# IGNF/MAESTRO

Hardware: AMD Instinct MI355X
Metric: MAE-pretrain tiles/sec (higher is better)
Workload: dtype bf16

## Files before the change

### maestro_amd/csrc/gemm.hip

```cpp
#include "gemm_reg.hpp"

namespace {

template <bool A_KMAJOR, bool B_KMAJOR, int MT = 4>
__global__ __launch_bounds__(NT, MT == 2 ? 3 : 2) void gemm_kernel(GemmParams p) {
    static_assert(!A_KMAJOR || MT == 4, "the K-major A image is 128 columns wide");
    constexpr int TBM = 32 * MT, NA = MT;
    constexpr int A_BYTES = TBM * 128, B_BYTES = TILE_BYTES;
    __shared__ __attribute__((aligned(16))) unsigned char smem[2 * A_BYTES + 2 * B_BYTES];
    unsigned char* const sb = smem + 2 * A_BYTES;
    const int nwg = p.tiles_m * p.tiles_n;
    const int id = xcd_remap(blockIdx.x, nwg);
    constexpr int GROUP_M = MT == 2 ? 16 : 8;
    int tile_m, tile_n;
    raster_tile<GROUP_M>(p, id, tile_m, tile_n);
    const int m0 = tile_m * TBM, n0 = tile_n * BN;
    const int kbeg = blockIdx.y * p.k_per_split;
    const int kend = min(p.K, kbeg + p.k_per_split);
    const int nk = (kend - kbeg + BK - 1) / BK;

    const int w = threadIdx.x >> 6, l = threadIdx.x & 63;
    const int wm = (w >> 1) * (16 * MT), wn = (w & 1) * 64;

    f32x4 acc[4][MT];
#pragma unroll
    for (int j = 0; j < 4; ++j)
#pragma unroll
        for (int i = 0; i < MT; ++i) acc[j][i] = (f32x4){0.f, 0.f, 0.f, 0.f};

    u32x4 ra[NA], rb[4];
    auto mfma_block = [&](const bf16x8 (&fa)[MT], const bf16x8 (&fb)[4]) {
#pragma unroll
        for (int j = 0; j < 4; ++j)
#pragma unroll
            for (int i = 0; i < MT; ++i)
                acc[j][i] = __builtin_amdgcn_mfma_f32_16x16x32_bf16(fb[j], fa[i], acc[j][i], 0, 0, 0);
    };
    auto compute = [&](const unsigned char* ta, const unsigned char* tb) {
#pragma unroll
        for (int s = 0; s < 2; ++s) {
            bf16x8 fa[MT], fb[4];
#pragma unroll
            for (int i = 0; i < MT; ++i) fa[i] = read_frag<A_KMAJOR>(ta, wm + 16 * i, s);
#pragma unroll
            for (int j = 0; j < 4; ++j) fb[j] = read_frag<B_KMAJOR>(tb, wn + 16 * j, s);
            mfma_block(fa, fb);
        }
    };
    auto compute_half = [&](const unsigned char* ta, const unsigned char* tb, int s) {
        bf16x8 fa[MT], fb[4];
#pragma unroll
        for (int i = 0; i < MT; ++i) fa[i] = read_frag<A_KMAJOR>(ta, wm + 16 * i, s);
#pragma unroll
        for (int j = 0; j < 4; ++j) fb[j] = read_frag<B_KMAJOR>(tb, wn + 16 * j, s);
        __builtin_amdgcn_s_setprio(1);
        mfma_block(fa, fb);
        __builtin_amdgcn_s_setprio(0);
    };
    if (p.fast) {
        const __amdgpu_buffer_rsrc_t ra_src = buffer_rsrc(p.A, (int)p.a_bytes);
        const __amdgpu_buffer_rsrc_t rb_src = buffer_rsrc(p.B, (int)p.b_bytes);
        int va[NA], vb[4];
        tile_offsets<A_KMAJOR, NA>(p.lda, m0, va);
        tile_offsets<B_KMAJOR>(p.ldb, n0, vb);
        const int a_step = A_KMAJOR ? BK * p.lda * 2 : BK * 2;
        const int b_step = B_KMAJOR ? BK * p.ldb * 2 : BK * 2;
        int a_off = A_KMAJOR ? kbeg * p.lda * 2 : kbeg * 2;
        int b_off = B_KMAJOR ? kbeg * p.ldb * 2 : kbeg * 2;
        load_tile_fast(ra_src, va, a_off, ra);
        load_tile_fast(rb_src, vb, b_off, rb);
        store_tile<A_KMAJOR, NA>(smem, ra);
        store_tile<B_KMAJOR>(sb, rb);
        if (nk > 1) {
            a_off += a_step; b_off += b_step;
            load_tile_fast(ra_src, va, a_off, ra);
            load_tile_fast(rb_src, vb, b_off, rb);
        }
        __syncthreads();
        constexpr int NM = 4 * MT, NS = NA + 4;
        constexpr int NR = (A_KMAJOR ? 8 : MT) + (B_KMAJOR ? 8 : 4);
        int kt0 = 0;
        for (; kt0 + 2 < nk; ++kt0) {
            const int cur = kt0 & 1;
            const unsigned char* ta = smem + cur * A_BYTES;
            const unsigned char* tb = sb + cur * B_BYTES;
            bf16x8 fa[MT], fb[4];
#pragma unroll
            for (int i = 0; i < MT; ++i) fa[i] = read_frag<A_KMAJOR>(ta, wm + 16 * i, 0);
#pragma unroll
            for (int j = 0; j < 4; ++j) fb[j] = read_frag<B_KMAJOR>(tb, wn + 16 * j, 0);
            mfma_block(fa, fb);
            store_tile<A_KMAJOR, NA>(smem + (cur ^ 1) * A_BYTES, ra);
            store_tile<B_KMAJOR>(sb + (cur ^ 1) * B_BYTES, rb);
            a_off += a_step; b_off += b_step;
            load_tile_fast(ra_src, va, a_off, ra);
            load_tile_fast(rb_src, vb, b_off, rb);
#pragma unroll
            for (int i = 0; i < MT; ++i) fa[i] = read_frag<A_KMAJOR>(ta, wm + 16 * i, 1);
#pragma unroll
            for (int j = 0; j < 4; ++j) fb[j] = read_frag<B_KMAJOR>(tb, wn + 16 * j, 1);
            mfma_block(fa, fb);
            __builtin_amdgcn_sched_group_barrier(0x100, NR, 0);
#pragma unroll
            for (int r = 0; r < NS; ++r) {
                __builtin_amdgcn_sched_group_barrier(0x008, NM / NS, 0);
                __builtin_amdgcn_sched_group_barrier(0x200, 1, 0);
                __builtin_amdgcn_sched_group_barrier(0x020, 1, 0);
            }
            if constexpr (NM % NS != 0) __builtin_amdgcn_sched_group_barrier(0x008, NM - (NM / NS) * NS, 0);
            __builtin_amdgcn_sched_group_barrier(0x100, NR, 0);
            __builtin_amdgcn_sched_group_barrier(0x008, NM, 0);
            __syncthreads();
        }
        for (int kt = kt0; kt < nk; ++kt) {
            const int cur = kt & 1;
            const unsigned char* ta = smem + cur * A_BYTES;
            const unsigned char* tb = sb + cur * B_BYTES;
            compute_half(ta, tb, 0);
            if (kt + 1 < nk) {
                store_tile<A_KMAJOR, NA>(smem + (cur ^ 1) * A_BYTES, ra);
                store_tile<B_KMAJOR>(sb + (cur ^ 1) * B_BYTES, rb);
                if (kt + 2 < nk) {
                    a_off += a_step; b_off += b_step;
                    load_tile_fast(ra_src, va, a_off, ra);
                    load_tile_fast(rb_src, vb, b_off, rb);
                }
            }
            compute_half(ta, tb, 1);
            __syncthreads();
        }
    } else {
        unsigned char* ta = smem;
        unsigned char* tb = sb;
        load_tile<A_KMAJOR, NA>(p.A, p.lda, m0, p.M, kbeg, kend, ra);
        load_tile<B_KMAJOR>(p.B, p.ldb, n0, p.N, kbeg, kend, rb);
        store_tile<A_KMAJOR, NA>(ta, ra);
        store_tile<B_KMAJOR>(tb, rb);
        __syncthreads();
        for (int kt = 0; kt < nk; ++kt) {
            const bool more = kt + 1 < nk;
            if (more) {
                load_tile<A_KMAJOR, NA>(p.A, p.lda, m0, p.M, kbeg + (kt + 1) * BK, kend, ra);
                load_tile<B_KMAJOR>(p.B, p.ldb, n0, p.N, kbeg + (kt + 1) * BK, kend, rb);
            }
            compute(ta, tb);
            __syncthreads();
            if (more) {
                store_tile<A_KMAJOR, NA>(ta, ra);
                store_tile<B_KMAJOR>(tb, rb);
            }
            __syncthreads();
        }
    }

    float* st = reinterpret_cast<float*>(smem) + w * (32 * 68);
    if (p.flags & MH_GEMM_ATOMIC) gemm_epilogue_atomic<MT>(p, acc, st, m0 + wm, n0 + wn);
    else gemm_epilogue_store<MT>(p, acc, st, m0 + wm, n0 + wn);
}

}

static int gemm_reg_launch(int tile, int layout, GemmParams& p, hipStream_t s) {
    const int K = p.K;
    const int mt = tile == MH_TILE_REG_64 ? 2 : tile == MH_TILE_REG_192 ? 6 : 4;
    const int tbm = 32 * mt;
    p.tiles_m = ceil_div(p.M, tbm); p.tiles_n = ceil_div(p.N, BN);
    const int ksteps = ceil_div(K, BK);
    const SplitK sk = (p.flags & MH_GEMM_ATOMIC) ? split_k(p.tiles_m * p.tiles_n, ksteps, 512, 4) : SplitK{ksteps, 1};
    p.k_per_split = sk.ksteps_per * BK;
    const bool a_kmajor = layout == 2, b_kmajor = layout != 0;
    const long k_rows = (long)ksteps * BK;
    const bool tail_ok = (a_kmajor && b_kmajor) || K % BK == 0;
    p.fast = tail_ok && gemm_in_reach((a_kmajor ? k_rows : (long)p.tiles_m * tbm) * p.lda * 2, 4096) &&
             gemm_in_reach((b_kmajor ? k_rows : (long)p.tiles_n * BN) * p.ldb * 2, 4096);
    gemm_set_extents(p, layout);
    dim3 grid(p.tiles_m * p.tiles_n, sk.splits), block(NT);
    for_layout(layout, [&](auto a_kmajor_c, auto b_kmajor_c) {
        constexpr bool AK = decltype(a_kmajor_c)::value, BKM = decltype(b_kmajor_c)::value;
        if (AK || mt == 4) hipLaunchKernelGGL((gemm_kernel<AK, BKM, 4>), grid, block, 0, s, p);
        else if (mt == 2) hipLaunchKernelGGL((gemm_kernel<false, BKM, 2>), grid, block, 0, s, p);
        else hipLaunchKernelGGL((gemm_kernel<false, BKM, 6>), grid, block, 0, s, p);
    });
    MH_LAUNCH_CHECK();
    return 0;
}

static int gemm_check_args(bool buffers, int tile, int layout, const GemmParams& p) {
    const int M = p.M, N = p.N, K = p.K, lda = p.lda, ldb = p.ldb, ldc = p.ldc, ldr = p.ldr, ldaux = p.ldaux, flags = p.flags;
    auto given = [&](const void* q) { return !buffers || q; };
    MH_CHECK_ARG(tile >= MH_TILE_AUTO && tile <= MH_TILE_REG_192, "mh_gemm_bf16: tile %d", tile);
    MH_CHECK_ARG(layout >= 0 && layout <= 2, "mh_gemm_bf16: layout %d", layout);
    MH_CHECK_ARG(!(flags & ~0x7ff), "mh_gemm_bf16: unknown flag bits 0x%x", flags & ~0x7ff);
    MH_CHECK_ARG(M > 0 && N > 0 && K > 0, "mh_gemm_bf16: empty problem %d %d %d", M, N, K);
    MH_CHECK_ARG(given(p.A) && given(p.B) && given(p.C), "mh_gemm_bf16: null operand");
    MH_CHECK_ARG(lda % 8 == 0 && ldb % 8 == 0, "mh_gemm_bf16: lda/ldb must be multiples of 8 (%d, %d)", lda, ldb);
    MH_CHECK_ARG(N % 4 == 0 && ldc % 4 == 0, "mh_gemm_bf16: N and ldc must be multiples of 4 (%d, %d)", N, ldc);
    MH_CHECK_ARG((flags & MH_GEMM_OUT_F32) || (N % 8 == 0 && ldc % 8 == 0), "mh_gemm_bf16: bf16 output needs N, ldc %% 8 == 0");
    MH_CHECK_ARG((flags & MH_GEMM_OUT_F32) || !(flags & MH_GEMM_RESIDUAL), "mh_gemm_bf16: residual epilogue needs f32 output");
    MH_CHECK_ARG(!(flags & MH_GEMM_OUT_F32) || !(flags & (MH_GEMM_GELU | MH_GEMM_DGELU | MH_GEMM_MULAUX)), "mh_gemm_bf16: GELU / aux epilogues need bf16 output");
    MH_CHECK_ARG(((uintptr_t)p.A | (uintptr_t)p.B | (uintptr_t)p.C) % 16 == 0, "mh_gemm_bf16: bases must be 16-B aligned");
    if (layout == 2) {
        MH_CHECK_ARG(M % 8 == 0 && N % 8 == 0, "mh_gemm_bf16: TN needs M, N multiples of 8 (%d, %d)", M, N);
    } else {
        MH_CHECK_ARG(K % 8 == 0, "mh_gemm_bf16: K must be a multiple of 8 (%d)", K);
        if (layout == 1) MH_CHECK_ARG(N % 8 == 0, "mh_gemm_bf16: NN needs N multiple of 8 (%d)", N);
    }
    MH_CHECK_ARG(!(flags & MH_GEMM_BIAS) || given(p.bias), "mh_gemm_bf16: bias flag without pointer");
    MH_CHECK_ARG(!(flags & MH_GEMM_RESIDUAL) || (given(p.res) && ldr % 4 == 0), "mh_gemm_bf16: residual needs pointer, ldr%%4==0");
    MH_CHECK_ARG(!(flags & (MH_GEMM_DGELU | MH_GEMM_MULAUX)) || (given(p.aux_in) && ldaux % 8 == 0), "mh_gemm_bf16: dgelu / mulaux need aux_in, ldaux %% 8 == 0");
    MH_CHECK_ARG(!(flags & MH_GEMM_AUX_DGELU) || ((flags & MH_GEMM_GELU) && given(p.aux_out)), "mh_gemm_bf16: aux_dgelu needs the GELU epilogue and aux_out");
    MH_CHECK_ARG(!((flags & MH_GEMM_DGELU) && (flags & MH_GEMM_MULAUX)), "mh_gemm_bf16: dgelu and mulaux exclude each other");
    MH_CHECK_ARG(!(flags & MH_GEMM_AUX_U8) || ((flags & (MH_GEMM_AUX_DGELU | MH_GEMM_MULAUX)) && !(flags & MH_GEMM_DGELU)),
                 "mh_gemm_bf16: MH_GEMM_AUX_U8 applies to the saved GELU derivative only (AUX_DGELU / MULAUX)");
    MH_CHECK_ARG(!(flags & MH_GEMM_GELU) || !p.aux_out || ldaux % 8 == 0, "mh_gemm_bf16: ldaux %% 8");
    MH_CHECK_ARG(!(flags & MH_GEMM_ATOMIC) || (flags & MH_GEMM_OUT_F32), "mh_gemm_bf16: atomic needs f32 output");
    MH_CHECK_ARG(!(flags & MH_GEMM_COLSUM) || (given(p.colsum) && !(flags & MH_GEMM_OUT_F32)), "mh_gemm_bf16: colsum needs a pointer and bf16 output");
    MH_CHECK_ARG(!(flags & MH_GEMM_ATOMIC) || !(flags & ~(MH_GEMM_ATOMIC | MH_GEMM_OUT_F32)),
                 "mh_gemm_bf16: atomic accumulate excludes other epilogues");
    return 0;
}

static bool prefer_dma(int layout, int M, int N, int K, int flags) {
    if (layout == 2 || (flags & MH_GEMM_ATOMIC) || K % 32 != 0 || K < 256) return false;
    const long tiles = (long)ceil_div(M, 256) * ceil_div(N, 256);
    if (tiles < 256) return false;
    const long waves = (tiles + 255) / 256;
    return 10 * tiles >= 9 * 256 * waves;
}

static int gemm_resolve(int tile, int families, int layout, const GemmParams& p) {
    const int M = p.M, N = p.N, K = p.K, flags = p.flags;
    if (tile >= MH_TILE_PP_128 && tile <= MH_TILE_PP_128_DIAG5) return gemm_pp_serves(tile, layout, p) ? tile : -2;
    if (tile > MH_TILE_REG_128 && tile < MH_TILE_PP_128) return gemm_dma_serves(tile, layout, p) ? tile : -2;
    if (tile != MH_TILE_AUTO)
        return layout != 2 && !(flags & MH_GEMM_COLSUM) ? tile : MH_TILE_REG_128;
    const bool dma = (families & MH_GEMM_FAMILY_DMA) && prefer_dma(layout, M, N, K, flags);
    const long t128 = (long)ceil_div(M, 128) * ceil_div(N, 128);
    if ((families & MH_GEMM_FAMILY_192) && !dma && layout != 2 && !(flags & (MH_GEMM_COLSUM | MH_GEMM_ATOMIC)) && K >= 1536 &&
        K % BK == 0 && t128 > 512 && t128 <= 576 && (long)ceil_div(M, 192) * ceil_div(N, 128) <= 512)
        return MH_TILE_REG_192;
    if ((families & MH_GEMM_FAMILY_PP) && !(flags & MH_GEMM_MULAUX) && layout == 0 && t128 >= 256 &&
        ((flags & MH_GEMM_GELU) ? t128 <= 2304 : (!dma || (K < 1024 && t128 <= 8192))) && gemm_pp_serves(MH_TILE_PP_128, layout, p))
        return MH_TILE_PP_128;
    if (dma && gemm_dma_serves(MH_TILE_DMA_256, layout, p)) return MH_TILE_DMA_256;
    return MH_TILE_REG_128;
}

extern "C" int mh_gemm_bf16_resolve_tile(int tile, int families, int layout, int M, int N, int K, int lda, int ldb, int ldc,
                                         int ldr, int ldaux, int flags) {
    GemmParams p;
    gemm_fill(p, M, N, K, nullptr, lda, nullptr, ldb, nullptr, ldc, flags, nullptr, nullptr, ldr, nullptr, nullptr, ldaux, nullptr);
    MH_CHECK_ARG(!(families & ~MH_GEMM_FAMILY_ALL), "mh_gemm_bf16_resolve_tile: unknown family bits 0x%x", families & ~MH_GEMM_FAMILY_ALL);
    if (const int rc = gemm_check_args(false, tile, layout, p)) return rc;
    return gemm_resolve(tile, families, layout, p);
}

extern "C" int mh_gemm_bf16_tile(int tile, int layout, int M, int N, int K, const void* A, int lda, const void* B, int ldb,
                                 void* C, int ldc, int flags, const float* bias, const float* res, int ldr,
                                 const void* aux_in, void* aux_out, int ldaux, float* colsum, void* stream) {
    GemmParams p;
    gemm_fill(p, M, N, K, A, lda, B, ldb, C, ldc, flags, bias, res, ldr, aux_in, aux_out, ldaux, colsum);
    if (const int rc = gemm_check_args(true, tile, layout, p)) return rc;
    const int run = gemm_resolve(tile, MH_GEMM_FAMILY_ALL, layout, p);
    if (run == -2) return -2;
    if (run >= MH_TILE_PP_128 && run <= MH_TILE_PP_128_DIAG5) return gemm_pp_launch(run, layout, p, (hipStream_t)stream);
    if (run > MH_TILE_REG_128 && run < MH_TILE_PP_128) return gemm_dma_launch(run, layout, p, (hipStream_t)stream);
    return gemm_reg_launch(run, layout, p, (hipStream_t)stream);
}

extern "C" int mh_gemm_bf16(int layout, int M, int N, int K, const void* A, int lda, const void* B, int ldb, void* C,
                            int ldc, int flags, const float* bias, const float* res, int ldr, const void* aux_in,
                            void* aux_out, int ldaux, float* colsum, void* stream) {
    return mh_gemm_bf16_tile(MH_TILE_AUTO, layout, M, N, K, A, lda, B, ldb, C, ldc, flags, bias, res, ldr, aux_in, aux_out,
                             ldaux, colsum, stream);
}
```

### maestro_amd/csrc/gemm_common.hpp

```cpp
#pragma once
#include "common.hpp"
#include "../../include/maestro_hip.h"

struct GemmParams {
    const bf16_t* A; const bf16_t* B; void* C;
    const float* bias; const float* res; const bf16_t* aux_in; bf16_t* aux_out; float* colsum;
    int M, N, K, lda, ldb, ldc, ldr, ldaux, flags;
    int tiles_m, tiles_n, k_per_split;
    int fast;
    unsigned a_bytes, b_bytes;
    const float* descale_a = nullptr; const float* descale_b = nullptr;
    uint8_t* c8 = nullptr; const float* c8_scale = nullptr; float* c8_amax = nullptr; int ldc8 = 0;
    const uint8_t* sa = nullptr; const uint8_t* sb = nullptr; int ldsa = 0, ldsb = 0; unsigned sa_bytes = 0, sb_bytes = 0;
    uint8_t* c8_scales = nullptr; int ldc8s = 0;
};

__device__ __forceinline__ __amdgpu_buffer_rsrc_t buffer_rsrc(const void* ptr, int bytes) {
    return __builtin_amdgcn_make_buffer_rsrc((void*)ptr, (short)0, bytes, 0x00020000);
}
__host__ __device__ __forceinline__ long matrix_bytes(int rows, int cols, int ld, int esize) { return ((long)(rows - 1) * ld + cols) * esize; }
__device__ __forceinline__ void swap16(uint32_t& a, uint32_t& b) {
    const u32x2 r = __builtin_amdgcn_permlane16_swap(a, b, false, false);
    a = r[0]; b = r[1];
}
template <int N>
__device__ __forceinline__ void wait_vmcnt() { asm volatile("s_waitcnt vmcnt(%0)" ::"n"(N) : "memory"); }
__device__ __forceinline__ int lane_id() { return __builtin_amdgcn_mbcnt_hi(~0u, __builtin_amdgcn_mbcnt_lo(~0u, 0u)); }
__device__ __forceinline__ int lane_id_opaque() {
    int lane = lane_id();
    asm volatile("" : "+v"(lane));
    return lane;
}
__device__ __forceinline__ int kmajor_sw(int k) { return (k & 3) | (((k >> 3) & 1) << 2); }

template <int GROUP_M>
__device__ __forceinline__ void raster_tile(const GemmParams& p, int id, int& tile_m, int& tile_n) {
    const int per_group = GROUP_M * p.tiles_n;
    const int group = id / per_group, in_group = id - group * per_group;
    const int first_m = group * GROUP_M;
    const int gsz = min(p.tiles_m - first_m, GROUP_M);
    tile_m = first_m + in_group % gsz;
    int n = in_group / gsz;
    const int groups = (p.tiles_m + GROUP_M - 1) / GROUP_M;
    n += ((group * 8) / groups) * p.tiles_n / 8;
    tile_n = n >= p.tiles_n ? n - p.tiles_n : n;
}

__device__ __forceinline__ u32x2 pack_fp8x8(f32x4 lo, f32x4 hi, float s, bool e5m2 = false) {
    const float lim = e5m2 ? 57344.f : 448.f;
#pragma unroll
    for (int e = 0; e < 4; ++e) {
        lo[e] = fminf(fmaxf(lo[e] * s, -lim), lim);
        hi[e] = fminf(fmaxf(hi[e] * s, -lim), lim);
    }
    int a, b;
    if (e5m2) {
        a = __builtin_amdgcn_cvt_pk_bf8_f32(lo[0], lo[1], 0, false);
        a = __builtin_amdgcn_cvt_pk_bf8_f32(lo[2], lo[3], a, true);
        b = __builtin_amdgcn_cvt_pk_bf8_f32(hi[0], hi[1], 0, false);
        b = __builtin_amdgcn_cvt_pk_bf8_f32(hi[2], hi[3], b, true);
    } else {
        a = __builtin_amdgcn_cvt_pk_fp8_f32(lo[0], lo[1], 0, false);
        a = __builtin_amdgcn_cvt_pk_fp8_f32(lo[2], lo[3], a, true);
        b = __builtin_amdgcn_cvt_pk_fp8_f32(hi[0], hi[1], 0, false);
        b = __builtin_amdgcn_cvt_pk_fp8_f32(hi[2], hi[3], b, true);
    }
    return (u32x2){(uint32_t)a, (uint32_t)b};
}
__device__ __forceinline__ uint32_t pack_e4m3x4(f32x4 v, float s) {
#pragma unroll
    for (int e = 0; e < 4; ++e) v[e] = fminf(fmaxf(v[e] * s, -448.f), 448.f);
    int a = __builtin_amdgcn_cvt_pk_fp8_f32(v[0], v[1], 0, false);
    a = __builtin_amdgcn_cvt_pk_fp8_f32(v[2], v[3], a, true);
    return (uint32_t)a;
}
__device__ __forceinline__ uint32_t mx_scale_byte(float a) {
    const uint32_t u = __float_as_uint(a);
    if (u >= 0x7f800000u) return 0xffu;
    if (u == 0u) return 127u;
    const int eb = (int)(u >> 23);
    const int b = eb - 8 + ((u & 0x7fffffu) > 0x600000u ? 1 : 0);
    return eb == 0 ? 0u : (uint32_t)max(b, 0);
}
__device__ __forceinline__ float mx_inv_scale(uint32_t byte) { return byte == 0xffu ? 1.f : __uint_as_float((254u - byte) << 23); }
template <int LANES>
__device__ __forceinline__ float group_amax(float v) {
    uint32_t u = __float_as_uint(v);
#pragma unroll
    for (int o = 1; o < LANES; o <<= 1) u = max(u, (uint32_t)__shfl_xor((int)u, o, 64));
    return __uint_as_float(u);
}

__device__ __forceinline__ void atomic_max_pos(float* row, float v) {
    const unsigned k = ((blockIdx.x + blockIdx.y * gridDim.x) * (blockDim.x >> 6) + (threadIdx.x >> 6)) & (MH_FP8_AMAX_SUBSLOTS - 1);
    __hip_atomic_fetch_max(reinterpret_cast<int*>(row) + k * MH_FP8_AMAX_STRIDE, __float_as_int(v), __ATOMIC_RELAXED,
                           __HIP_MEMORY_SCOPE_AGENT);
}

__host__ __device__ static inline void gemm_fill(GemmParams& p, int M, int N, int K, const void* A, int lda, const void* B, int ldb, void* C, int ldc,
                             int flags, const float* bias, const float* res, int ldr, const void* aux_in, void* aux_out, int ldaux,
                             float* colsum) {
    p.A = (const bf16_t*)A; p.B = (const bf16_t*)B; p.C = C;
    p.bias = bias; p.res = res; p.aux_in = (const bf16_t*)aux_in; p.aux_out = (bf16_t*)aux_out; p.colsum = colsum;
    p.M = M; p.N = N; p.K = K; p.lda = lda; p.ldb = ldb; p.ldc = ldc; p.ldr = ldr; p.ldaux = ldaux; p.flags = flags;
}
__host__ __device__ static inline long gemm_extent(bool kmajor, int rows, int K, int ld, int esize = 2) {
    return kmajor ? matrix_bytes(K, rows, ld, esize) : matrix_bytes(rows, K, ld, esize);
}
static inline void gemm_set_extents(GemmParams& p, int layout) {
    p.a_bytes = (unsigned)gemm_extent(layout == 2, p.M, p.K, p.lda);
    p.b_bytes = (unsigned)gemm_extent(layout != 0, p.N, p.K, p.ldb);
}
static inline bool gemm_in_reach(long bytes, long margin = 65536) { return bytes < (1L << 31) - margin; }
struct SplitK { int ksteps_per, splits; };
static inline SplitK split_k(int tiles, int ksteps, int slots, int min_ksteps) {
    const int want = max(1, min(min(slots / max(tiles, 1), ksteps / min_ksteps), 32));
    const int ksteps_per = ceil_div(ksteps, want);
    return {ksteps_per, ceil_div(ksteps, ksteps_per)};
}
template <class F>
static void for_layout(int layout, F&& fn) {
    using std::false_type; using std::true_type;
    switch (layout) {
        case 0: fn(false_type{}, false_type{}); break;
        case 1: fn(false_type{}, true_type{}); break;
        default: fn(true_type{}, true_type{}); break;
    }
}

bool gemm_dma_serves(int tile, int layout, const GemmParams& p);
int gemm_dma_launch(int tile, int layout, GemmParams& p, hipStream_t stream);
bool gemm_pp_serves(int tile, int layout, const GemmParams& p);
int gemm_pp_launch(int tile, int layout, GemmParams& p, hipStream_t stream);

__device__ __forceinline__ u32x2 pack_dgelu_u8x8(f32x4 lo, f32x4 hi) {
    unsigned a = 0, b = 0;
#pragma unroll
    for (int e = 0; e < 4; ++e) {
        a = __builtin_amdgcn_cvt_pk_u8_f32(__builtin_fmaf(lo[e], 200.f, 26.f), e, a);
        b = __builtin_amdgcn_cvt_pk_u8_f32(__builtin_fmaf(hi[e], 200.f, 26.f), e, b);
    }
    return (u32x2){a, b};
}
__device__ __forceinline__ f32x4 unpack_dgelu_u8x4(unsigned w) {
    return (f32x4){__builtin_fmaf((float)(w & 0xffu), 0.005f, -0.13f), __builtin_fmaf((float)((w >> 8) & 0xffu), 0.005f, -0.13f),
                   __builtin_fmaf((float)((w >> 16) & 0xffu), 0.005f, -0.13f), __builtin_fmaf((float)(w >> 24), 0.005f, -0.13f)};
}

template <int MT, int RP = 32, bool MX = false>
__device__ __forceinline__ void gemm_epilogue_store(const GemmParams& p, const f32x4 (&acc)[4][MT], float* st, int m_base,
                                                    int n_base) {
    constexpr int TPP = RP / 16, NPASS = MT / TPP, SUB = RP / 8;
    static_assert((RP == 16 || RP == 32) && MT % TPP == 0, "staging pass geometry");
    const int l = threadIdx.x & 63, g = l >> 4, lm = l & 15;
    const bool out_f32 = p.flags & MH_GEMM_OUT_F32;
    const float alpha = p.descale_a ? *p.descale_a * *p.descale_b : 1.f;
    if (out_f32) {
        f32x4 bias4[4];
#pragma unroll
        for (int j = 0; j < 4; ++j) {
            const int n = n_base + 16 * j + 4 * g;
            bias4[j] = (f32x4){0, 0, 0, 0};
            if ((p.flags & MH_GEMM_BIAS) && n < p.N) bias4[j] = *reinterpret_cast<const f32x4*>(p.bias + n);
        }
        constexpr int IB = MT % 4 == 0 ? 4 : MT % 3 == 0 ? 3 : MT;
        static_assert(MT % IB == 0, "row blocks per wave");
#pragma unroll
        for (int i0 = 0; i0 < MT; i0 += IB) {
            f32x4 add[IB][4];
#pragma unroll
            for (int ii = 0; ii < IB; ++ii) {
                const int m = m_base + 16 * (i0 + ii) + lm;
#pragma unroll
                for (int j = 0; j < 4; ++j) {
                    const int n = n_base + 16 * j + 4 * g;
                    add[ii][j] = bias4[j];
                    if ((p.flags & MH_GEMM_RESIDUAL) && m < p.M && n < p.N)
                        add[ii][j] += *reinterpret_cast<const f32x4*>(p.res + (size_t)m * p.ldr + n);
                }
            }
#pragma unroll
            for (int ii = 0; ii < IB; ++ii) {
                const int m = m_base + 16 * (i0 + ii) + lm;
#pragma unroll
                for (int j = 0; j < 4; ++j) {
                    const int n = n_base + 16 * j + 4 * g;
                    if (m < p.M && n < p.N)
                        *reinterpret_cast<f32x4*>(reinterpret_cast<float*>(p.C) + (size_t)m * p.ldc + n) = acc[j][i0 + ii] * alpha + add[ii][j];
                }
            }
        }
        return;
    }
    f32x4 cs_lo = {0, 0, 0, 0}, cs_hi = {0, 0, 0, 0};
    float s8 = 0.f;
    if constexpr (!MX) s8 = p.c8 ? *p.c8_scale : 0.f;
    float amax8 = 0.f;
    u32x4 aux_all[NPASS][SUB];
    {
        const int n = n_base + (l & 7) * 8;
        if (p.flags & (MH_GEMM_DGELU | MH_GEMM_MULAUX)) {
#pragma unroll
            for (int pass_m = 0; pass_m < NPASS; ++pass_m)
#pragma unroll
                for (int pass = 0; pass < SUB; ++pass) {
                    const int m = m_base + RP * pass_m + pass * 8 + (l >> 3);
                    aux_all[pass_m][pass] = (u32x4){0, 0, 0, 0};
                    if (m < p.M && n < p.N) {
                        if (p.flags & MH_GEMM_AUX_U8) {
                            const u32x2 b8 = *reinterpret_cast<const u32x2*>(reinterpret_cast<const uint8_t*>(p.aux_in) + (size_t)m * p.ldaux + n);
                            aux_all[pass_m][pass] = (u32x4){b8[0], b8[1], 0, 0};
                        } else {
                            aux_all[pass_m][pass] = *reinterpret_cast<const u32x4*>(p.aux_in + (size_t)m * p.ldaux + n);
                        }
                    }
                }
        }
    }
#pragma unroll
    for (int pass_m = 0; pass_m < NPASS; ++pass_m) {
#pragma unroll
        for (int i = TPP * pass_m; i < TPP * pass_m + TPP; ++i)
#pragma unroll
            for (int j = 0; j < 4; ++j)
                *reinterpret_cast<f32x4*>(st + (16 * (i - TPP * pass_m) + lm) * 68 + 16 * j + 4 * g) = acc[j][i];
        {
            const int c = (l & 7) * 8, n = n_base + c;
            f32x4 b_lo = {0, 0, 0, 0}, b_hi = {0, 0, 0, 0};
            if ((p.flags & MH_GEMM_BIAS) && n < p.N) {
                b_lo = *reinterpret_cast<const f32x4*>(p.bias + n);
                b_hi = *reinterpret_cast<const f32x4*>(p.bias + n + 4);
            }
            const u32x4 (&aux_pre)[SUB] = aux_all[pass_m];
#pragma unroll
            for (int pass = 0; pass < SUB; ++pass) {
                const int r = pass * 8 + (l >> 3), m = m_base + RP * pass_m + r;
                f32x4 lo = *reinterpret_cast<const f32x4*>(st + r * 68 + c);
                f32x4 hi = *reinterpret_cast<const f32x4*>(st + r * 68 + c + 4);
                if (m < p.M && n < p.N) {
                    if (p.descale_a) { lo = lo * alpha + b_lo; hi = hi * alpha + b_hi; }
                    else { lo += b_lo; hi += b_hi; }
                    if (p.flags & MH_GEMM_GELU) {
                        f32x4 c_lo, d_lo, c_hi, d_hi;
                        gelu_cdf_pdf4(lo, c_lo, d_lo);
                        gelu_cdf_pdf4(hi, c_hi, d_hi);
                        if (p.aux_out) {
                            f32x4 a_lo = lo, a_hi = hi;
                            if (p.flags & MH_GEMM_AUX_DGELU) { a_lo = lo * d_lo + c_lo; a_hi = hi * d_hi + c_hi; }
                            if (p.flags & MH_GEMM_AUX_U8) {
                                *reinterpret_cast<u32x2*>(reinterpret_cast<uint8_t*>(p.aux_out) + (size_t)m * p.ldaux + n) =
                                    pack_dgelu_u8x8(a_lo, a_hi);
                            } else {
                                u32x4 pk = {pack_bf2(a_lo[0], a_lo[1]), pack_bf2(a_lo[2], a_lo[3]), pack_bf2(a_hi[0], a_hi[1]),
                                            pack_bf2(a_hi[2], a_hi[3])};
                                *reinterpret_cast<u32x4*>(p.aux_out + (size_t)m * p.ldaux + n) = pk;
                            }
                        }
                        lo *= c_lo; hi *= c_hi;
                    }
                    if (p.flags & MH_GEMM_MULAUX) {
                        const u32x4 pk = aux_pre[pass];
                        if (p.flags & MH_GEMM_AUX_U8) {
                            lo *= unpack_dgelu_u8x4(pk[0]);
                            hi *= unpack_dgelu_u8x4(pk[1]);
                        } else {
                            lo *= bf2x2_to_f32x4(pk[0], pk[1]);
                            hi *= bf2x2_to_f32x4(pk[2], pk[3]);
                        }
                    }
                    if (p.flags & MH_GEMM_DGELU) {
                        const u32x4 pk = aux_pre[pass];
                        const f32x4 h_lo = {__uint_as_float(pk[0] << 16), __uint_as_float(pk[0] & 0xffff0000u),
                                            __uint_as_float(pk[1] << 16), __uint_as_float(pk[1] & 0xffff0000u)};
                        const f32x4 h_hi = {__uint_as_float(pk[2] << 16), __uint_as_float(pk[2] & 0xffff0000u),
                                            __uint_as_float(pk[3] << 16), __uint_as_float(pk[3] & 0xffff0000u)};
                        lo *= gelu_erf_grad4(h_lo);
                        hi *= gelu_erf_grad4(h_hi);
                    }
                    if (p.flags & MH_GEMM_COLSUM) { cs_lo += lo; cs_hi += hi; }
                    u32x4 pk = {pack_bf2(lo[0], lo[1]), pack_bf2(lo[2], lo[3]), pack_bf2(hi[0], hi[1]), pack_bf2(hi[2], hi[3])};
                    *reinterpret_cast<u32x4*>(reinterpret_cast<bf16_t*>(p.C) + (size_t)m * p.ldc + n) = pk;
                    if (p.c8) {
                        if constexpr (MX) {
                            const f32x4 qlo = bf2x2_to_f32x4(pk[0], pk[1]), qhi = bf2x2_to_f32x4(pk[2], pk[3]);
                            float a = 0.f;
#pragma unroll
                            for (int e = 0; e < 4; ++e) a = amax_fold(amax_fold(a, qlo[e]), qhi[e]);
                            const uint32_t sbyte = mx_scale_byte(group_amax<4>(a));
                            const float inv = mx_inv_scale(sbyte);
                            *reinterpret_cast<u32x2*>(p.c8 + (size_t)m * p.ldc8 + n) = (u32x2){pack_e4m3x4(qlo, inv), pack_e4m3x4(qhi, inv)};
                            if ((l & 3) == 0) p.c8_scales[(size_t)m * p.ldc8s + (n >> 5)] = (uint8_t)sbyte;
                        } else {
                            *reinterpret_cast<u32x2*>(p.c8 + (size_t)m * p.ldc8 + n) = pack_fp8x8(lo, hi, s8, p.flags & MH_GEMM_C8_E5M2);
#pragma unroll
                            for (int e = 0; e < 4; ++e) amax8 = amax_fold(amax_fold(amax8, lo[e]), hi[e]);
                        }
                    }
                }
            }
            if ((p.flags & MH_GEMM_COLSUM) && (RP * (pass_m + 1)) % 64 == 0) {
#pragma unroll
                for (int o = 8; o < 64; o <<= 1) {
#pragma unroll
                    for (int e = 0; e < 4; ++e) {
                        cs_lo[e] += __shfl_xor(cs_lo[e], o, 64);
                        cs_hi[e] += __shfl_xor(cs_hi[e], o, 64);
                    }
                }
                const int m_blk = m_base + RP * (pass_m + 1) - 64;
                if (l < 8 && n < p.N && m_blk < p.M) {
                    float* dst = p.colsum + (size_t)(m_blk >> 6) * p.N + n;
                    *reinterpret_cast<f32x4*>(dst) = cs_lo;
                    *reinterpret_cast<f32x4*>(dst + 4) = cs_hi;
                }
                cs_lo = (f32x4){0, 0, 0, 0}; cs_hi = (f32x4){0, 0, 0, 0};
            }
        }
    }
    if (!MX && p.c8 && p.c8_amax) {
        amax8 = wave_amax(amax8);
        if (l == 0 && amax_nonzero(amax8)) atomic_max_pos(p.c8_amax, amax8);
    }
}

template <int MT>
__device__ __forceinline__ void gemm_epilogue_atomic(const GemmParams& p, const f32x4 (&acc)[4][MT], float* st, int m_base,
                                                     int n_base) {
    const int l = threadIdx.x & 63, g = l >> 4, lm = l & 15;
#pragma unroll
    for (int pass_m = 0; pass_m < MT / 2; ++pass_m) {
#pragma unroll
        for (int i = 2 * pass_m; i < 2 * pass_m + 2; ++i)
#pragma unroll
            for (int j = 0; j < 4; ++j)
#pragma unroll
                for (int r = 0; r < 4; ++r) st[(16 * (i - 2 * pass_m) + lm) * 65 + 16 * j + 4 * g + r] = acc[j][i][r];
        const int n = n_base + l;
        if (n < p.N) {
            for (int rr = 0; rr < 32; ++rr) {
                const int m = m_base + 32 * pass_m + rr;
                if (m < p.M) atomicAdd(reinterpret_cast<float*>(p.C) + (size_t)m * p.ldc + n, st[rr * 65 + l]);
            }
        }
    }
}
```

Before: 1804.

## Prefetch GEMM epilogue bias/residual/aux operands during final K iterations

Adds an EpiOperands register struct and a request function that loads bias, residual and aux tensors into registers before the last K-tile compute, so their global-memory latency overlaps MFMA work instead of stalling the epilogue. The fast path's tail loop is peeled into two explicit iterations (now requiring nk>1), and single-tile cases fall back to the generic path. This raises register pressure, which may reduce occupancy or cause spills.

```diff
diff --git a/maestro_amd/csrc/gemm.hip b/maestro_amd/csrc/gemm.hip
--- a/maestro_amd/csrc/gemm.hip
+++ b/maestro_amd/csrc/gemm.hip
@@ -29,6 +29,8 @@
         for (int i = 0; i < MT; ++i) acc[j][i] = (f32x4){0.f, 0.f, 0.f, 0.f};
 
     u32x4 ra[NA], rb[4];
+    EpiOperands<MT> pre;
+    const bool prefetch = !(p.flags & MH_GEMM_ATOMIC);
     auto mfma_block = [&](const bf16x8 (&fa)[MT], const bf16x8 (&fb)[4]) {
 #pragma unroll
         for (int j = 0; j < 4; ++j)
@@ -57,7 +59,7 @@
         mfma_block(fa, fb);
         __builtin_amdgcn_s_setprio(0);
     };
-    if (p.fast) {
+    if (p.fast && nk > 1) {
         const __amdgpu_buffer_rsrc_t ra_src = buffer_rsrc(p.A, (int)p.a_bytes);
         const __amdgpu_buffer_rsrc_t rb_src = buffer_rsrc(p.B, (int)p.b_bytes);
         int va[NA], vb[4];
@@ -71,11 +73,9 @@
         load_tile_fast(rb_src, vb, b_off, rb);
         store_tile<A_KMAJOR, NA>(smem, ra);
         store_tile<B_KMAJOR>(sb, rb);
-        if (nk > 1) {
-            a_off += a_step; b_off += b_step;
-            load_tile_fast(ra_src, va, a_off, ra);
-            load_tile_fast(rb_src, vb, b_off, rb);
-        }
+        a_off += a_step; b_off += b_step;
+        load_tile_fast(ra_src, va, a_off, ra);
+        load_tile_fast(rb_src, vb, b_off, rb);
         __syncthreads();
         constexpr int NM = 4 * MT, NS = NA + 4;
         constexpr int NR = (A_KMAJOR ? 8 : MT) + (B_KMAJOR ? 8 : 4);
@@ -112,20 +112,22 @@
             __builtin_amdgcn_sched_group_barrier(0x008, NM, 0);
             __syncthreads();
         }
-        for (int kt = kt0; kt < nk; ++kt) {
-            const int cur = kt & 1;
+        {
+            const int cur = kt0 & 1;
             const unsigned char* ta = smem + cur * A_BYTES;
             const unsigned char* tb = sb + cur * B_BYTES;
             compute_half(ta, tb, 0);
-            if (kt + 1 < nk) {
-                store_tile<A_KMAJOR, NA>(smem + (cur ^ 1) * A_BYTES, ra);
-                store_tile<B_KMAJOR>(sb + (cur ^ 1) * B_BYTES, rb);
-                if (kt + 2 < nk) {
-                    a_off += a_step; b_off += b_step;
-                    load_tile_fast(ra_src, va, a_off, ra);
-                    load_tile_fast(rb_src, vb, b_off, rb);
-                }
-            }
+            store_tile<A_KMAJOR, NA>(smem + (cur ^ 1) * A_BYTES, ra);
+            store_tile<B_KMAJOR>(sb + (cur ^ 1) * B_BYTES, rb);
+            if (prefetch) gemm_epilogue_request<MT>(p, m0 + wm, n0 + wn, pre);
+            compute_half(ta, tb, 1);
+            __syncthreads();
+        }
+        {
+            const int cur = (kt0 + 1) & 1;
+            const unsigned char* ta = smem + cur * A_BYTES;
+            const unsigned char* tb = sb + cur * B_BYTES;
+            compute_half(ta, tb, 0);
             compute_half(ta, tb, 1);
             __syncthreads();
         }
@@ -151,11 +153,12 @@
             }
             __syncthreads();
         }
+        if (prefetch) gemm_epilogue_request<MT>(p, m0 + wm, n0 + wn, pre);
     }
 
     float* st = reinterpret_cast<float*>(smem) + w * (32 * 68);
     if (p.flags & MH_GEMM_ATOMIC) gemm_epilogue_atomic<MT>(p, acc, st, m0 + wm, n0 + wn);
-    else gemm_epilogue_store<MT>(p, acc, st, m0 + wm, n0 + wn);
+    else gemm_epilogue_store<MT, 32, false, true>(p, acc, st, m0 + wm, n0 + wn, &pre);
 }
 
 }
diff --git a/maestro_amd/csrc/gemm_common.hpp b/maestro_amd/csrc/gemm_common.hpp
--- a/maestro_amd/csrc/gemm_common.hpp
+++ b/maestro_amd/csrc/gemm_common.hpp
@@ -147,9 +147,67 @@
                    __builtin_fmaf((float)((w >> 16) & 0xffu), 0.005f, -0.13f), __builtin_fmaf((float)(w >> 24), 0.005f, -0.13f)};
 }
 
-template <int MT, int RP = 32, bool MX = false>
+template <int MT, int RP = 32>
+struct EpiOperands {
+    static constexpr int IB = MT % 4 == 0 ? 4 : MT % 3 == 0 ? 3 : MT;
+    static constexpr int NAUX = (MT / (RP / 16)) * (RP / 8);
+    u32x4 w[4 * IB > NAUX ? 4 * IB : NAUX];
+    f32x4 bias[4];
+};
+template <int MT, int RP = 32>
+__device__ __forceinline__ void gemm_epilogue_request(const GemmParams& p, int m_base, int n_base, EpiOperands<MT, RP>& o) {
+    constexpr int IB = EpiOperands<MT, RP>::IB, NPASS = MT / (RP / 16), SUB = RP / 8;
+    const int l = threadIdx.x & 63, g = l >> 4, lm = l & 15;
+    if (p.flags & MH_GEMM_OUT_F32) {
+#pragma unroll
+        for (int j = 0; j < 4; ++j) {
+            const int n = n_base + 16 * j + 4 * g;
+            o.bias[j] = (f32x4){0, 0, 0, 0};
+            if ((p.flags & MH_GEMM_BIAS) && n < p.N) o.bias[j] = *reinterpret_cast<const f32x4*>(p.bias + n);
+        }
+#pragma unroll
+        for (int ii = 0; ii < IB; ++ii) {
+            const int m = m_base + 16 * ii + lm;
+#pragma unroll
+            for (int j = 0; j < 4; ++j) {
+                const int n = n_base + 16 * j + 4 * g;
+                o.w[ii * 4 + j] = (u32x4){0, 0, 0, 0};
+                if ((p.flags & MH_GEMM_RESIDUAL) && m < p.M && n < p.N)
+                    o.w[ii * 4 + j] = *reinterpret_cast<const u32x4*>(p.res + (size_t)m * p.ldr + n);
+            }
+        }
+        return;
+    }
+    const int n = n_base + (l & 7) * 8;
+    o.bias[0] = (f32x4){0, 0, 0, 0}; o.bias[1] = (f32x4){0, 0, 0, 0};
+    if ((p.flags & MH_GEMM_BIAS) && n < p.N) {
+        o.bias[0] = *reinterpret_cast<const f32x4*>(p.bias + n);
+        o.bias[1] = *reinterpret_cast<const f32x4*>(p.bias + n + 4);
+    }
+    if (!(p.flags & (MH_GEMM_DGELU | MH_GEMM_MULAUX))) return;
+    if (p.flags & MH_GEMM_AUX_U8) {
+#pragma unroll
+        for (int k = 0; k < NPASS * SUB; ++k) {
+            const int m = m_base + k * 8 + (l >> 3);
+            o.w[k] = (u32x4){0, 0, 0, 0};
+            if (m < p.M && n < p.N) {
+                const u32x2 b8 = *reinterpret_cast<const u32x2*>(reinterpret_cast<const uint8_t*>(p.aux_in) + (size_t)m * p.ldaux + n);
+                o.w[k] = (u32x4){b8[0], b8[1], 0, 0};
+            }
+        }
+    } else {
+#pragma unroll
+        for (int k = 0; k < NPASS * SUB; ++k) {
+            const int m = m_base + k * 8 + (l >> 3);
+            o.w[k] = (u32x4){0, 0, 0, 0};
+            if (m < p.M && n < p.N) o.w[k] = *reinterpret_cast<const u32x4*>(p.aux_in + (size_t)m * p.ldaux + n);
+        }
+    }
+}
+
+template <int MT, int RP = 32, bool MX = false, bool PRE = false>
 __device__ __forceinline__ void gemm_epilogue_store(const GemmParams& p, const f32x4 (&acc)[4][MT], float* st, int m_base,
-                                                    int n_base) {
+                                                    int n_base, const EpiOperands<MT, RP>* pre = nullptr) {
     constexpr int TPP = RP / 16, NPASS = MT / TPP, SUB = RP / 8;
     static_assert((RP == 16 || RP == 32) && MT % TPP == 0, "staging pass geometry");
     const int l = threadIdx.x & 63, g = l >> 4, lm = l & 15;
@@ -160,10 +218,14 @@
 #pragma unroll
         for (int j = 0; j < 4; ++j) {
             const int n = n_base + 16 * j + 4 * g;
-            bias4[j] = (f32x4){0, 0, 0, 0};
-            if ((p.flags & MH_GEMM_BIAS) && n < p.N) bias4[j] = *reinterpret_cast<const f32x4*>(p.bias + n);
-        }
-        constexpr int IB = MT % 4 == 0 ? 4 : MT % 3 == 0 ? 3 : MT;
+            if constexpr (PRE) {
+                bias4[j] = pre->bias[j];
+            } else {
+                bias4[j] = (f32x4){0, 0, 0, 0};
+                if ((p.flags & MH_GEMM_BIAS) && n < p.N) bias4[j] = *reinterpret_cast<const f32x4*>(p.bias + n);
+            }
+        }
+        constexpr int IB = EpiOperands<MT, RP>::IB;
         static_assert(MT % IB == 0, "row blocks per wave");
 #pragma unroll
         for (int i0 = 0; i0 < MT; i0 += IB) {
@@ -175,8 +237,10 @@
                 for (int j = 0; j < 4; ++j) {
                     const int n = n_base + 16 * j + 4 * g;
                     add[ii][j] = bias4[j];
-                    if ((p.flags & MH_GEMM_RESIDUAL) && m < p.M && n < p.N)
-                        add[ii][j] += *reinterpret_cast<const f32x4*>(p.res + (size_t)m * p.ldr + n);
+                    if ((p.flags & MH_GEMM_RESIDUAL) && m < p.M && n < p.N) {
+                        if (PRE && i0 == 0) add[ii][j] += __builtin_bit_cast(f32x4, pre->w[ii * 4 + j]);
+                        else add[ii][j] += *reinterpret_cast<const f32x4*>(p.res + (size_t)m * p.ldr + n);
+                    }
                 }
             }
 #pragma unroll
@@ -199,7 +263,12 @@
     u32x4 aux_all[NPASS][SUB];
     {
         const int n = n_base + (l & 7) * 8;
-        if (p.flags & (MH_GEMM_DGELU | MH_GEMM_MULAUX)) {
+        if constexpr (PRE) {
+#pragma unroll
+            for (int pass_m = 0; pass_m < NPASS; ++pass_m)
+#pragma unroll
+                for (int pass = 0; pass < SUB; ++pass) aux_all[pass_m][pass] = pre->w[pass_m * SUB + pass];
+        } else if (p.flags & (MH_GEMM_DGELU | MH_GEMM_MULAUX)) {
 #pragma unroll
             for (int pass_m = 0; pass_m < NPASS; ++pass_m)
 #pragma unroll
@@ -227,7 +296,9 @@
         {
             const int c = (l & 7) * 8, n = n_base + c;
             f32x4 b_lo = {0, 0, 0, 0}, b_hi = {0, 0, 0, 0};
-            if ((p.flags & MH_GEMM_BIAS) && n < p.N) {
+            if constexpr (PRE) {
+                b_lo = pre->bias[0]; b_hi = pre->bias[1];
+            } else if ((p.flags & MH_GEMM_BIAS) && n < p.N) {
                 b_lo = *reinterpret_cast<const f32x4*>(p.bias + n);
                 b_hi = *reinterpret_cast<const f32x4*>(p.bias + n + 4);
             }
```

Result: no change. 1810, median of 6 (+0.4%).
